# fatimp/SIFT3D

Measured on AMD Instinct MI355X. Metric: Mvoxel/s detect+describe (float32 volume resident in HBM), higher is better.
Workload: dtype f32; 1 GPU; 512x512x512 float32 lattice-blob volume, detect+describe, default parameters (sigma0 1.6, sigma_n 1.15, 3 levels/octave); parallelism=single GPU

## Files before the change

include/sift3d_amd.h:

```cpp
#ifndef SIFT3D_AMD_H
#define SIFT3D_AMD_H

#include <stddef.h>
#include <stdint.h>

#include "sift3d/imtypes.h"

#ifdef __cplusplus
extern "C" {
#endif

#define SIFT3D_AMD_API __attribute__((visibility("default")))


SIFT3D_AMD_API int
sift3d_amd_detect_keypoints_device(sift3d_detector *det, const float *d_volume,
                                   int nx, int ny, int nz, double ux, double uy,
                                   double uz, sift3d_keypoint_store *store);

SIFT3D_AMD_API int
sift3d_amd_image_set_units(sift3d_image *im, double ux, double uy, double uz);

SIFT3D_AMD_API int
sift3d_amd_detector_set_cuboid_extrema(sift3d_detector *det, int on);
// ... 659 lines not shown
                           float *d_R, int32_t *d_keep, void *d_tab, uint32_t max_cand, int slot, void *stream);

typedef struct {
    float R[9];
    float cx, cy, cz;
    int32_t level;
    uint32_t row1;
    double sd;
} sift3d_hip_kp;

SIFT3D_AMD_API int
sift3d_hip_describe(const sift3d_hip_level *d_levels, const sift3d_hip_kp *d_kp,
                    uint32_t n, float *d_hist, void *stream);

SIFT3D_AMD_API size_t sift3d_hip_describe_wlut_floats(int nlevels);
SIFT3D_AMD_API int
sift3d_hip_describe_wlut(const sift3d_hip_level *d_levels, int nlevels, const sift3d_hip_kp *d_kp,
                         uint32_t n, float *d_hist, float *d_wlut, void *stream);
SIFT3D_AMD_API size_t sift3d_hip_describe_part_bytes(uint32_t n);
SIFT3D_AMD_API int
sift3d_hip_describe_parts(const sift3d_hip_level *d_levels, int nlevels, const sift3d_hip_kp *d_kp,
                          uint32_t n, uint32_t n_exact, float *d_hist, float *d_hist2, float *d_wlut,
                          void *d_part, void *stream);
SIFT3D_AMD_API int
sift3d_hip_describe_clock(const float *d_wlut, int nlevels, int exact, uint64_t *cycles, uint64_t *ticks,
                          void *stream);
SIFT3D_AMD_API int
sift3d_hip_describe_wlut2(const sift3d_hip_level *d_levels, int nlevels, const sift3d_hip_kp *d_kp,
                          uint32_t n, float *d_hist, float *d_hist2, float *d_wlut, void *stream);
SIFT3D_AMD_API int
sift3d_hip_describe_ex(const sift3d_hip_level *d_levels, int nlevels, const sift3d_hip_kp *d_kp, uint32_t n,
                       uint32_t n_exact, float *d_hist, float *d_hist2, float *d_wlut, void *stream);

SIFT3D_AMD_API int sift3d_hip_slab_count(const sift3d_hip_cand *d_cand, const int32_t *d_keep, uint32_t n,
                                         int ngl, int K, int nkey, int32_t *d_cnt, void *stream);
SIFT3D_AMD_API size_t sift3d_hip_slab_pack_scratch_bytes(uint32_t n);
SIFT3D_AMD_API int sift3d_hip_slab_pack(const sift3d_hip_level *d_levels, const sift3d_hip_cand *d_cand,
                                        const int32_t *d_keep, const float *d_R, uint32_t n, int ngl,
                                        float *d_vals, void *d_recs, void *d_scratch, void *stream);
SIFT3D_AMD_API int sift3d_hip_slab_build(const void *d_all, size_t blk_bytes, size_t roff, size_t toff,
                                         int world, int nkey, const uint32_t *d_tab, uint32_t tot_k,
                                         uint32_t tot_c, void *d_out, void *stream);

#define SIFT3D_HIP_FACE_FLOATS 19
SIFT3D_AMD_API int
sift3d_hip_set_mesh(const float *faces );
// ... 18 lines not shown
```

sift3d_amd/csrc/sift3d_describe.hip:

```cpp
#include "sift3d_kernels_common.h"
#include "sift3d_math.h"

#include <algorithm>
#include <cmath>
#include <cstdlib>

struct FaceRec {
    float v0[3], e1[3], e2[3], t[3], q[3], e2q, idx[3];
};
static_assert(sizeof(FaceRec) == SIFT3D_HIP_FACE_FLOATS * 4, "face record layout");

__constant__ float c_face16[20 * 16];
__constant__ int c_bin_off[12];
__constant__ int c_oct_face[32];

constexpr int DQ = 256;
constexpr int HIST_USED = 800;
constexpr int HIST_LDS = 800;
constexpr int FACE_STRIDE = 20;
constexpr int RSUPER = 68;
constexpr int REC_FLOATS = 7 * RSUPER;
constexpr int rec_row(int r) { return r < 7 ? r * RSUPER : (r - 7) * RSUPER + 32; }
constexpr int rec_group(int r) { return (rec_row(r) / 4) % 16; }
constexpr bool rec_groups_distinct()
// ... 86 lines not shown
    int e;
    const float mant = frexpf(L.ux, &e);
    const float u2 = L.ux * L.ux;
    const bool ok = L.ux == L.uy && L.ux == L.uz && mant == 0.5f &&
                    rad2 / u2 < (float)(WL_STRIDE - WL_HEAD - 1) && u2 * (float)WL_STRIDE < 16777216.0f;
    if (threadIdx.x == 0) {
        tab[0] = ok ? 1.0f : 0.0f;
        tab[1] = 0.0f;
        tab[2] = __int_as_float((int)(__double_as_longlong(L.sd) & 0xffffffffll));
        tab[3] = __int_as_float((int)(__double_as_longlong(L.sd) >> 32));
    }
    if (!ok)
        return;
    for (int k = threadIdx.x; k < WL_STRIDE - WL_HEAD; k += 256) {
        const float sq = (float)k * u2;
        const float arg = -0.5f * sq / sig2;
        tab[WL_HEAD + k] = arg >= -150.0f ? s3d_expf(arg) : 0.0f;
    }
}

constexpr int DWAVES = 4;
constexpr int DPARTS = 4;

template <bool EXACT>
__global__ __launch_bounds__(64 * DWAVES) void k_describe(const sift3d_hip_level *__restrict__ levels,
                                                 const sift3d_hip_kp *__restrict__ kps, uint32_t first,
                                                 uint32_t n,
                                                 float *__restrict__ out, float *__restrict__ out2,
                                                 const float *__restrict__ wlut,
                                                 uint32_t *__restrict__ work, float *__restrict__ part,
                                                 uint32_t *__restrict__ done DESC_ABLATE_ARG)
{
    __shared__ float hist_[DWAVES][2 * HIST_LDS];
    __shared__ __attribute__((aligned(16))) float rec_[DWAVES][REC_FLOATS];
    __shared__ int queue_[DWAVES][DQ];
    __shared__ __attribute__((aligned(16))) float sface[20 * FACE_STRIDE];
    __shared__ int soct[32];
    __shared__ uint64_t sexp[32];
    const int wv = __builtin_amdgcn_readfirstlane((int)(threadIdx.x >> 6));
    const int lane = threadIdx.x & 63;
    float *const hist = hist_[wv];
    float *const rec = rec_[wv];
    const uint32_t rec_m0 = (uint32_t)__builtin_amdgcn_readfirstlane((int)lds_addr(rec));
    const uint32_t hist_m0 = (uint32_t)__builtin_amdgcn_readfirstlane((int)lds_addr(hist));
    int *const queue = queue_[wv];
    for (int i = threadIdx.x; i < 20 * 16; i += 64 * DWAVES)
        sface[(i >> 4) * FACE_STRIDE + (i & 15)] = c_face16[i];
    if (threadIdx.x < 32) {
        soct[threadIdx.x] = c_oct_face[threadIdx.x];
        sexp[threadIdx.x] = s3d_exp2_tab[threadIdx.x];
    }
    __syncthreads();
    const bool probe = work && blockIdx.x == 0 && threadIdx.x == 0;
    long long probe_c0 = 0, probe_w0 = 0;
    if (probe) {
        probe_c0 = clock64();
        probe_w0 = wall_clock64();
    }
    const bool split = !EXACT && part != nullptr;
    for (bool first_pass = true;; first_pass = false) {
    uint32_t item;
    if (work) {
        uint32_t t = 0;
        if (lane == 0)
            t = atomicAdd(work, 1u);
        item = (uint32_t)__builtin_amdgcn_readfirstlane((int)t);
    } else {
        if (!first_pass)
            break;
        item = blockIdx.x * DWAVES + wv;
    }
    const uint32_t ki = first + (split ? item / DPARTS : item);
    const int pp = split ? (int)(item % DPARTS) : 0;
    if (ki >= n)
        break;
    static_assert(2 * HIST_LDS == 25 * 64, "histogram clear: 25 whole-wave stores");
#define Z4(o) "ds_write_addtid_b32 %0 offset:" #o "\n\tds_write_addtid_b32 %0 offset:" #o "+256\n\t" \
              "ds_write_addtid_b32 %0 offset:" #o "+512\n\tds_write_addtid_b32 %0 offset:" #o "+768\n\t"
    asm volatile("s_mov_b32 m0, %1\n\ts_nop 0\n\t" Z4(0) Z4(1024) Z4(2048) Z4(3072) Z4(4096) Z4(5120)
                 "ds_write_addtid_b32 %0 offset:6144" ::"v"(0.0f), "s"(hist_m0) : "m0", "memory");
#undef Z4
    wave_sync();
    const sift3d_hip_kp K = kps[ki];
    const sift3d_hip_level L = levels[K.level];
    const uint32_t orow = K.row1 ? K.row1 - 1 : ki;
    const float *__restrict__ wtab = nullptr;
    const int icx = (int)K.cx, icy = (int)K.cy, icz = (int)K.cz;
    if (wlut) {
        const float *tab = wlut + (size_t)K.level * WL_STRIDE;
        const long long sdbits = ((long long)__float_as_int(tab[3]) << 32) | (unsigned)__float_as_int(tab[2]);
        if (tab[0] == 1.0f && sdbits == __double_as_longlong(K.sd) && (float)icx == K.cx &&
            (float)icy == K.cy && (float)icz == K.cz)
            wtab = tab + WL_HEAD;
    }

    typedef const float __attribute__((address_space(1))) *gfloat_p;
    const gfloat_p wsrc = wtab ? (gfloat_p)wtab : (gfloat_p) reinterpret_cast<const float *>(levels);
    const int wmask = wtab ? -1 : 0;

    const float sigma = (float)(K.sd * 7.071067812);
    const float rad = (float)(2.0 * (double)sigma);
    const float half_w = (float)((double)rad / 1.4142135623730951);
    const float desc_w = 2.0f * half_w;
    const float hist_w = desc_w / 4.0f;
    const float bin_f = 1.0f / hist_w;
    const float rad2 = rad * rad;
    const float sig2 = sigma * sigma;
    const float *R = K.R;
    const float iux = 1.0f / L.ux, iuy = 1.0f / L.uy, iuz = 1.0f / L.uz;
    Box B;
    bounds_f(K.cx, rad, L.ux, L.nx, B.xs, B.xe);
    bounds_f(K.cy, rad, L.uy, L.ny, B.ys, B.ye);
    bounds_f(K.cz, rad, L.uz, L.nz_glob, B.zs, B.ze);
    B.zs = max(B.zs, L.z_off + 1);
    B.ze = min(B.ze, L.z_off + L.nz - 2);
    const int xsh = 32 - __builtin_clz((unsigned)max(B.xe - B.xs, 1));
    const int ysh = xsh + 32 - __builtin_clz((unsigned)max(B.ye - B.ys, 1));
    const uint32_t xmask = (1u << xsh) - 1u, ymask = (1u << (ysh - xsh)) - 1u;
#if defined(__HIP_DEVICE_COMPILE__) && !defined(__gfx942__) && !defined(__gfx950__)
#error "k_describe's commit routes its factors with DPP quad_perm on wave64: validated on gfx942 / gfx950 only"
#endif
    const int half = lane >> 5, l5 = lane & 31;
    const int pc = l5 >> 2, pt = l5 & 3, pj = pt < 3 ? pt : 0;
    const int pxr = pt == 0 ? pc : 8 + pj;
    const int pdx = (pc >> 2) & 1, pdy = (pc >> 1) & 1, pdz = pc & 1;
    const int corner4 = 4 * (pdx + 4 * pdy + 16 * pdz);
    const int coff_a = corner4 + (EXACT ? (half == 0 ? 0 : HIST_LDS * 4) : half * (HIST_LDS * 4));
    const int coff_b = corner4 + (half == 1 ? 0 : HIST_LDS * 4);
    (void)coff_b;
    const unsigned long long lt_mask = (1ull << lane) - 1ull;

    uint32_t qhead = 0, qtail = 0;
    bool pend = false;
#ifdef SIFT3D_AMD_DIAG
    unsigned diag_voxels = 0;
#endif

    auto window = [&](int x, int y, int z, float &sq, float &vbx, float &vby, float &vbz) -> bool {
        const float dx = ((float)x - K.cx) * L.ux;
        const float dy = ((float)y - K.cy) * L.uy;
        const float dz = ((float)z - K.cz) * L.uz;
        sq = dx * dx + dy * dy + dz * dz;
        const float kx = R[0] * dx + R[3] * dy + R[6] * dz;
        const float ky = R[1] * dx + R[4] * dy + R[7] * dz;
        const float kz = R[2] * dx + R[5] * dy + R[8] * dz;
        vbx = (kx + half_w) * bin_f;
        vby = (ky + half_w) * bin_f;
        vbz = (kz + half_w) * bin_f;
        const float lo = fminf(fminf(vbx, vby), vbz), hi = fmaxf(fmaxf(vbx, vby), vbz);
        return !(sq > rad2) && !(lo < 0.0f) && !(hi >= 4.0f);
    };

    float pv[7] = { 0.f, 0.f, 0.f, 0.f, 0.f, 0.f, 0.f };
    int ppk = 0;
    const gfloat_p gdata = (gfloat_p)L.data;
    const uint32_t ys32 = (uint32_t)L.nx, zs32 = (uint32_t)L.nx * (uint32_t)L.ny;
    auto prefetch_loads = [&](uint32_t start, int cnt) {
        const int qv = queue[(start + lane) & (DQ - 1)];
        ppk = lane < cnt ? qv : ppk;
        const int x = B.xs + (int)((uint32_t)ppk & xmask), y = B.ys + (int)(((uint32_t)ppk >> xsh) & ymask),
                  zl = B.zs + (int)((uint32_t)ppk >> ysh) - L.z_off;
        const gfloat_p p = gdata + ((uint64_t)zs32 * (uint32_t)zl + (uint32_t)(x + (int)ys32 * y));
        pv[0] = p[1]; pv[1] = *(p - 1); pv[2] = p[ys32]; pv[3] = *(p - ys32);
        pv[4] = p[zs32]; pv[5] = *(p - zs32);
        if (wtab) {
            const int i = x - icx, j = y - icy, l = B.zs + (int)((uint32_t)ppk >> ysh) - icz;
            pv[6] = wtab[i * i + j * j + l * l];
        }
    };
    auto prefetch_weight = [&]() {
        if (wtab)
            return;
        const int x = B.xs + (int)((uint32_t)ppk & xmask), y = B.ys + (int)(((uint32_t)ppk >> xsh) & ymask);
        const float dx = ((float)x - K.cx) * L.ux;
        const float dy = ((float)y - K.cy) * L.uy;
        const float dz = ((float)(B.zs + (int)((uint32_t)ppk >> ysh)) - K.cz) * L.uz;
        pv[6] = s3d_expf_in_range(-0.5f * (dx * dx + dy * dy + dz * dz) / sig2, sexp);
    };
    auto prefetch = [&](uint32_t start, int cnt) {
        prefetch_loads(start, cnt);
        prefetch_weight();
    };

    float rp[2][7] = { { 0.f, 0.f, 0.f, 0.f, 0.f, 0.f, 0.f }, { 0.f, 0.f, 0.f, 0.f, 0.f, 0.f, 0.f } };
    const float *const xrd = rec + rec_row(pxr) + 16 * half;
    const int *const ard = reinterpret_cast<const int *>(rec + rec_row(11 + pj) + 16 * half);
    auto commit_write = [&](int pass) {
#define RS(i) "ds_write_addtid_b32 %" #i " offset:%c8*" #i "\n\t"
        asm volatile("s_mov_b32 m0, %7\n\ts_nop 0\n\t" RS(0) RS(1) RS(2) RS(3) RS(4) RS(5) RS(6)
                     ::"v"(rp[pass][0]), "v"(rp[pass][1]), "v"(rp[pass][2]), "v"(rp[pass][3]), "v"(rp[pass][4]),
                       "v"(rp[pass][5]), "v"(rp[pass][6]), "s"(rec_m0), "n"(RSUPER * 4)
                     : "m0", "memory");
#undef RS
        wave_sync();
    };
#define SB() __builtin_amdgcn_sched_barrier(0)
#ifndef DESC_OPT
#define DESC_OPT 7
#endif
#define QUAD_X(v) __int_as_float(__builtin_amdgcn_update_dpp(0, __float_as_int(v), 0x03, 0xf, 0xf, true))
#if DESC_OPT & 1
#define COMMIT_ADD(old, x) (EXACT ? (old) + QUAD_X(x) * (x) : quad_fmac(old, x))
#else
#define COMMIT_ADD(old, x) ((old) + QUAD_X(x) * (x))
#endif
#define KEEP(v) asm volatile("" ::"v"(v))
#define COMMIT_BEGIN(coff)                                                                    \
    const int coff4 = (coff);                                                                 \
    int4 cb4 = *reinterpret_cast<const int4 *>(ard);                                          \
    float4 cx4 = *reinterpret_cast<const float4 *>(xrd);                                      \
    int4 nb4 = cb4;                                                                           \
    float4 nx4 = cx4;
#define ROUND(u, ...)                                                                         \
    {                                                                                         \
        if (((u) & 3) == 0 && (u) + 4 < 16) {                                                 \
            nb4 = *reinterpret_cast<const int4 *>(ard + (u) + 4);                             \
            nx4 = *reinterpret_cast<const float4 *>(xrd + (u) + 4);                           \
        }                                                                                     \
        const int mb_[4] = { cb4.x, cb4.y, cb4.z, cb4.w };                                    \
        const float xv_[4] = { cx4.x, cx4.y, cx4.z, cx4.w };                                  \
        float *bin_ = reinterpret_cast<float *>(reinterpret_cast<char *>(hist) + (mb_[(u) & 3] + coff4)); \
        float old_ = 0.0f;                                                                    \
        if (!DESC_ABLATE(1))                                                                  \
            old_ = *bin_;                                                                     \
        SB();                                                                                 \
        { __VA_ARGS__ }                                                                       \
        SB();                                                                                 \
        if (!DESC_ABLATE(1))                                                                  \
            *bin_ = COMMIT_ADD(old_, xv_[(u) & 3]);                     \
        if (((u) & 3) == 3) {                                                                 \
            cb4 = nb4;                                                                        \
            cx4 = nx4;                                                                        \
        }                                                                                     \
        SB();                                                                                 \
    }
#define CHAIN_B()                                                                             \
    if (EXACT) {                                                                              \
        COMMIT_BEGIN(coff_b);                                                                 \
        ROUND(0, ) ROUND(1, ) ROUND(2, ) ROUND(3, ) ROUND(4, ) ROUND(5, ) ROUND(6, ) ROUND(7, ) \
        ROUND(8, ) ROUND(9, ) ROUND(10, ) ROUND(11, ) ROUND(12, ) ROUND(13, ) ROUND(14, ) ROUND(15, ) \
    }
    auto batch = [&](int cnt, const float *cv, int pk, uint32_t nstart, int ncnt) {
#ifdef SIFT3D_AMD_DIAG
        diag_voxels += (unsigned)cnt;
#endif
        if (DESC_ABLATE(2)) { prefetch(nstart, ncnt); return; }
        int x, y, z;
        float dx, dy, dz, kx, ky, kz, vbx, vby, vbz, gx, gy, gz, rx, ry, rz, m2;
        float t1, t2, t3, px, py, pz, det, di, kk;
        float4 A0, A1, A2, A3;
        int f0;
        bool live = false, found = false;
        int fidx = 0;
        float b0 = 0.f, b1 = 0.f, b2 = 0.f;
        commit_write(0);
        {
            COMMIT_BEGIN(coff_a);
            ROUND(0, x = B.xs + (int)((uint32_t)pk & xmask); y = B.ys + (int)(((uint32_t)pk >> xsh) & ymask);
                     z = B.zs + (int)((uint32_t)pk >> ysh);
                     dx = ((float)x - K.cx) * L.ux; KEEP(dx);)
            ROUND(1, dy = ((float)y - K.cy) * L.uy; dz = ((float)z - K.cz) * L.uz; KEEP(dy); KEEP(dz);
                     gx = 0.5f * (cv[0] - cv[1]); gy = 0.5f * (cv[2] - cv[3]); gz = 0.5f * (cv[4] - cv[5]);)
            ROUND(2, gx *= iux; gy *= iuy; gz *= iuz;
                     gx = gx * cv[6]; gy = gy * cv[6]; gz = gz * cv[6];)
            ROUND(3, kx = R[0] * dx + R[3] * dy + R[6] * dz; ky = R[1] * dx + R[4] * dy + R[7] * dz; KEEP(kx); KEEP(ky);)
            ROUND(4, kz = R[2] * dx + R[5] * dy + R[8] * dz;
                     vbx = (kx + half_w) * bin_f; vby = (ky + half_w) * bin_f; vbz = (kz + half_w) * bin_f;
                     KEEP(vbx); KEEP(vby); KEEP(vbz);)
            ROUND(5, rx = R[0] * gx + R[3] * gy + R[6] * gz; ry = R[1] * gx + R[4] * gy + R[7] * gz;)
            ROUND(6, rz = R[2] * gx + R[5] * gy + R[8] * gz; m2 = rx * rx + ry * ry + rz * rz;
                     live = lane < cnt && !(m2 < 1.1920928955078125e-06f);)
#if DESC_OPT & 2
            ROUND(7, const float g = 1.6180339887f, g2 = 2.6180339887f;
                     const float ax_ = fabsf(rx), ay_ = fabsf(ry), az_ = fabsf(rz);
                     t1 = __builtin_fmaf(g2, ay_, __builtin_fmaf(-g, az_, ax_));
                     t2 = __builtin_fmaf(g2, az_, __builtin_fmaf(-g, ax_, ay_));
                     t3 = __builtin_fmaf(g2, ax_, __builtin_fmaf(-g, ay_, az_));)
#else
            ROUND(7, const float g = 1.6180339887f, g2 = 2.6180339887f;
                     const float ax_ = fabsf(rx), ay_ = fabsf(ry), az_ = fabsf(rz);
                     t1 = ax_ + g2 * ay_ - g * az_; t2 = ay_ + g2 * az_ - g * ax_; t3 = az_ + g2 * ax_ - g * ay_;)
#endif
            ROUND(8, const int n1 = t1 < 0.0f, n2 = t2 < 0.0f, n3 = t3 < 0.0f;
                     const int cls = n1 + (1 - n1) * (2 * n2 + (1 - n2) * 3 * n3);
// ... 25 lines not shown
                    found = true;
                    open = false;
                }
                if (__ballot(open) == 0ull)
                    break;
            }
        }
        commit_write(1);
        {
            COMMIT_BEGIN(coff_a);
            int nx_, ny_, nzl_, qv_;
            gfloat_p np_;
            float mag, fx, fy, fz;
            int ix, iy, iz, cell4;
            float ax[2], ay[2], az[2], fld[14];
            ROUND(0, qv_ = queue[(nstart + lane) & (DQ - 1)];)
            ROUND(1, ppk = lane < ncnt ? qv_ : ppk;
                     nx_ = B.xs + (int)((uint32_t)ppk & xmask); ny_ = B.ys + (int)(((uint32_t)ppk >> xsh) & ymask);
                     nzl_ = B.zs + (int)((uint32_t)ppk >> ysh) - L.z_off;
                     np_ = gdata + ((uint64_t)zs32 * (uint32_t)nzl_ + (uint32_t)(nx_ + (int)ys32 * ny_));)
            ROUND(2, pv[0] = np_[1]; pv[1] = *(np_ - 1); pv[2] = np_[ys32]; pv[3] = *(np_ - ys32);)
            ROUND(3, pv[4] = np_[zs32]; pv[5] = *(np_ - zs32);
                     const int i = nx_ - icx; const int j = ny_ - icy; const int l = B.zs + (int)((uint32_t)ppk >> ysh) - icz;
                     pv[6] = wsrc[(i * i + j * j + l * l) & wmask];)
#if DESC_OPT & 2
            ROUND(4, mag = EXACT ? sqrtf(m2) : __builtin_amdgcn_sqrtf(m2);
                     mag = live && found ? mag : 0.0f;)
#else
            ROUND(4, mag = sqrtf(m2); mag = live && found ? mag : 0.0f;)
#endif
            ROUND(5, fx = vbx - floorf(vbx); fy = vby - floorf(vby); fz = vbz - floorf(vbz);
                     ix = (int)vbx; iy = (int)vby; iz = (int)vbz;)
            ROUND(6, const bool lx = ix >= 3; const bool ly = iy >= 3; const bool lz = iz >= 3;
                     ax[0] = lx ? 0.0f : 1.0f - fx; ax[1] = lx ? 1.0f - fx : fx;
                     ay[0] = ly ? 0.0f : 1.0f - fy; ay[1] = ly ? 1.0f - fy : fy;
                     az[0] = lz ? 0.0f : 1.0f - fz; az[1] = lz ? 1.0f - fz : fz;)
            ROUND(7, _Pragma("unroll") for (int c = 0; c < 4; c++)
                         fld[c] = mag * (ax[(c >> 2) & 1] * ay[(c >> 1) & 1] * az[c & 1]);)
            ROUND(8, _Pragma("unroll") for (int c = 4; c < 8; c++)
                         fld[c] = mag * (ax[(c >> 2) & 1] * ay[(c >> 1) & 1] * az[c & 1]);)
            ROUND(9, cell4 = 4 * (min(max(ix, 0), 2) + 4 * min(max(iy, 0), 2) + 16 * min(max(iz, 0), 2));
                     const bool ok = live && found;
                     fld[8] = ok ? b0 : 0.0f; fld[9] = ok ? b1 : 0.0f; fld[10] = ok ? b2 : 0.0f;)
            ROUND(10, _Pragma("unroll") for (int j = 0; j < 3; j++)
                          fld[11 + j] = __int_as_float(4 * ((fidx >> (10 * j)) & 1023) + cell4);)
            ROUND(11, _Pragma("unroll") for (int i = 0; i < 4; i++) {
                          const auto r = __builtin_amdgcn_permlane32_swap(__float_as_uint(fld[i]), __float_as_uint(fld[7 + i]), false, false);
// ... 87 lines not shown
            if (__builtin_expect(__ballot(cheap2(xx, yy, in0, in1)) != 0ull, 0)) {
                float sq, vbx, vby, vbz;
                in0 = window(pxs + xx, pys + yy, z, sq, vbx, vby, vbz);
                in1 = window(pxs + xx + 1, pys + yy, z, sq, vbx, vby, vbz);
            }
#else
            float sq, vbx, vby, vbz;
            bool in0 = window(pxs + xx, pys + yy, z, sq, vbx, vby, vbz);
            bool in1 = window(pxs + xx + 1, pys + yy, z, sq, vbx, vby, vbz);
#endif
            in0 = in0 && c0 + 2 * lane < ppe;
            in1 = in1 && c0 + 2 * lane < ppe && xx + 1 < pbx;
            const int pk0 = (int)((uint32_t)(ox + xx) | ((uint32_t)(oy + yy) << xsh) | ((uint32_t)(z - B.zs) << ysh));
            const int pk1 = pk0 + 1;
            xx += r128;
            yy += q128;
            if (xx >= pbe) {
                xx -= pbe;
                yy++;
            }
            const unsigned long long m0 = __ballot(in0), m1 = __ballot(in1);
            if ((m0 | m1) == 0ull)
                continue;
            const uint32_t before = (uint32_t)__popcll(m0 & lt_mask) + (uint32_t)__popcll(m1 & lt_mask);
            if (in0)
                queue[(qtail + before) & (DQ - 1)] = pk0;
            if (in1)
                queue[(qtail + before + (in0 ? 1u : 0u)) & (DQ - 1)] = pk1;
            qtail += (uint32_t)__popcll(m0) + (uint32_t)__popcll(m1);
            wave_sync();
            while (qtail - qhead >= 64) {
                if (pend) {
                    float cv[7];
#pragma unroll
                    for (int k = 0; k < 7; k++)
                        cv[k] = pv[k];
                    const int cpk = ppk;
                    batch(64, cv, cpk, qhead, 64);
                } else {
                    prefetch(qhead, 64);
                    pend = true;
                }
                qhead += 64;
            }
        }
    }
    {
// ... 68 lines not shown
            for (int o = 32; o > 0; o >>= 1)
                norm += __shfl_xor(norm, o, 64);
        }
        norm = sqrt(norm) + 2.220446049250313e-16;
        const float inv = (float)(1.0 / norm);
        wave_sync();
        for (int i = lane; i < HIST_USED; i += 64) {
            float el = hist[i] * inv;
            if (pass == 0)
                el = el < trunc ? el : trunc;
            hist[i] = el;
        }
        wave_sync();
    }
    for (int i = lane; i < 768; i += 64) {
        const float v = hist[c_bin_off[i % 12] + i / 12];
        out[(size_t)orow * 768 + i] = v;
        if (out2)
            out2[(size_t)orow * 768 + i] = v;
    }
    wave_sync();
    }
    if (probe) {
        unsigned long long *slot = reinterpret_cast<unsigned long long *>(work - (EXACT ? 0 : 1) + (EXACT ? 4 : 8));
        slot[0] = (unsigned long long)(clock64() - probe_c0);
        slot[1] = (unsigned long long)(wall_clock64() - probe_w0);
    }
}

__constant__ int c_face_vert[20];

constexpr int DB_TX = 64, DB_TY = 4;

__device__ __forceinline__ void dense_bin_one(const float *sface, const int *soct, const int *svert, float gx,
                                              float gy, float gz, float &w0, float &w1, float &w2, int &vid)
{
    const float m2 = gx * gx + gy * gy + gz * gz;
    w0 = 0.0f; w1 = 0.0f; w2 = 0.0f; vid = 0;
    if (m2 < 1.1920928955078125e-06f)
        return;
    float b0, b1, b2;
    int fi, f = soct[icos_guess(gx, gy, gz)];
    bool found = face_eval(reinterpret_cast<const float4 *>(sface + f * FACE_STRIDE), gx, gy, gz, b0, b1, b2, fi) &&
                 fminf(b0, fminf(b1, b2)) > 2e-5f;
    if (!found) {
        for (f = 0; f < 20; f++)
            if (face_eval(reinterpret_cast<const float4 *>(sface + f * FACE_STRIDE), gx, gy, gz, b0, b1, b2, fi)) {
// ... 515 lines not shown
static unsigned describe_grid(uint32_t count, bool counted)
{
    const unsigned need = (count + DWAVES - 1) / DWAVES;
    if (!counted)
        return need;
    static int cus = 0;
    if (!cus) {
        int dev = 0;
        hipDeviceProp_t prop;
        if (hipGetDevice(&dev) == hipSuccess && hipGetDeviceProperties(&prop, dev) == hipSuccess)
            cus = prop.multiProcessorCount;
        if (cus < 1)
            cus = 256;
    }
    const unsigned cap = (unsigned)cus * 4u;
    return need < cap ? need : cap;
}

size_t sift3d_hip_describe_part_bytes(uint32_t n)
{
    return n ? (size_t)n * DPARTS * HIST_USED * sizeof(float) + (size_t)n * sizeof(uint32_t) : 0;
}

static int describe_launch(const sift3d_hip_level *d_levels, int nlevels, const sift3d_hip_kp *d_kp, uint32_t n,
                           uint32_t n_exact, float *d_hist, float *d_hist2, const float *d_wlut,
                           void *d_part, void *stream)
{
    if (n_exact > n)
        n_exact = n;
#ifdef SIFT3D_AMD_DIAG
    static int ablate = getenv("SIFT3D_AMD_DESC_ABLATE") ? atoi(getenv("SIFT3D_AMD_DESC_ABLATE")) : 0;
#define DESC_ABLATE_PASS , ablate
#else
#define DESC_ABLATE_PASS
#endif
    uint32_t *work = d_wlut ? reinterpret_cast<uint32_t *>(const_cast<float *>(d_wlut) + (size_t)nlevels * WL_STRIDE)
                            : nullptr;
    if (n_exact) {
        hipLaunchKernelGGL(k_describe<true>, dim3(describe_grid(n_exact, work != nullptr)), dim3(64 * DWAVES), 0,
                           (hipStream_t)stream, d_levels, d_kp, 0u, n_exact, d_hist, d_hist2, d_wlut,
                           work, (float *)nullptr, (uint32_t *)nullptr DESC_ABLATE_PASS);
        LAUNCH_CHECK();
    }
    if (n > n_exact) {
        const uint32_t nf = n - n_exact;
        void *tmp = nullptr;
        if (!d_part) {
            HIPCHK(hipMalloc(&tmp, sift3d_hip_describe_part_bytes(nf)));
            d_part = tmp;
        }
        float *parts = reinterpret_cast<float *>(d_part);
        uint32_t *done = reinterpret_cast<uint32_t *>(parts + (size_t)nf * DPARTS * HIST_USED);
        hipError_t e = hipMemsetAsync(done, 0, (size_t)nf * sizeof(uint32_t), (hipStream_t)stream);
        if (e == hipSuccess) {
            hipLaunchKernelGGL(k_describe<false>, dim3(describe_grid(nf * DPARTS, work != nullptr)),
                               dim3(64 * DWAVES), 0, (hipStream_t)stream, d_levels, d_kp, n_exact, n, d_hist,
                               d_hist2, d_wlut, work ? work + 1 : nullptr, parts, done DESC_ABLATE_PASS);
            e = hipGetLastError();
        }
        if (tmp) {
            const hipError_t e2 = hipStreamSynchronize((hipStream_t)stream);
            (void)hipFree(tmp);
            if (e == hipSuccess)
                e = e2;
        }
        if (e != hipSuccess)
            return fail("k_describe", e, __FILE__, __LINE__);
    }
#undef DESC_ABLATE_PASS
    return SIFT3D_SUCCESS;
}

int sift3d_hip_describe(const sift3d_hip_level *d_levels, const sift3d_hip_kp *d_kp, uint32_t n,
                        float *d_hist, void *stream)
{
    if (!n)
        return SIFT3D_SUCCESS;
    return describe_launch(d_levels, 0, d_kp, n, 0, d_hist, nullptr, nullptr, nullptr, stream);
}

int sift3d_hip_describe_parts(const sift3d_hip_level *d_levels, int nlevels, const sift3d_hip_kp *d_kp,
                              uint32_t n, uint32_t n_exact, float *d_hist, float *d_hist2, float *d_wlut,
                              void *d_part, void *stream)
{
    if (!n)
        return SIFT3D_SUCCESS;
    if (!d_wlut || nlevels < 1)
        return describe_launch(d_levels, 0, d_kp, n, n_exact, d_hist, d_hist2, nullptr, d_part, stream);
    hipLaunchKernelGGL(k_desc_wlut, dim3(nlevels), dim3(256), 0, (hipStream_t)stream, d_levels, nlevels,
                       d_wlut);
    return describe_launch(d_levels, nlevels, d_kp, n, n_exact, d_hist, d_hist2, d_wlut, d_part, stream);
}

int sift3d_hip_describe_ex(const sift3d_hip_level *d_levels, int nlevels, const sift3d_hip_kp *d_kp,
                           uint32_t n, uint32_t n_exact, float *d_hist, float *d_hist2, float *d_wlut,
                           void *stream)
{
    return sift3d_hip_describe_parts(d_levels, nlevels, d_kp, n, n_exact, d_hist, d_hist2, d_wlut, nullptr,
                                     stream);
}

int sift3d_hip_describe_clock(const float *d_wlut, int nlevels, int exact, uint64_t *cycles, uint64_t *ticks,
                              void *stream)
{
    if (!d_wlut || nlevels < 1 || !cycles || !ticks)
        return SIFT3D_FAILURE;
    uint64_t v[2] = { 0, 0 };
    const uint32_t *ctr = reinterpret_cast<const uint32_t *>(d_wlut + (size_t)nlevels * WL_STRIDE);
    HIPCHK(hipMemcpyAsync(v, ctr + (exact ? 4 : 8), sizeof(v), hipMemcpyDeviceToHost, (hipStream_t)stream));
    HIPCHK(hipStreamSynchronize((hipStream_t)stream));
    *cycles = v[0];
    *ticks = v[1];
    return SIFT3D_SUCCESS;
}
// ... 131 lines not shown
```

sift3d_amd/csrc/sift3d_detect.c:

```c

static int require_device(void)
{
    if (!sift3d_amd_device_available()) {
        ERR("sift3d_amd: no HIP device is available; this library has no CPU path \n");
        return SIFT3D_FAILURE;
    }
    return SIFT3D_SUCCESS;
}

static int ensure_device(sift3d_detector *d)
{
    int i;
    if (d->stream) {
        if (sift3d_hip_current_device() != d->device) {
            ERR("sift3d_amd: this detector belongs to HIP device %d, the current device is %d \n",
                d->device, sift3d_hip_current_device());
            return SIFT3D_FAILURE;
        }
        return SIFT3D_SUCCESS;
    }
    if (require_device())
        return SIFT3D_FAILURE;
    d->device = sift3d_hip_current_device();
    if (!(d->stream = sift3d_hip_stream_create()) || !(d->oct_stream = sift3d_hip_stream_create_high()) ||
// ... 791 lines not shown
    return SIFT3D_SUCCESS;
}

enum { DESC_LV_MAX = 32 };

static int ensure_kp_list(sift3d_detector *d, int num)
{
    if ((uint32_t)num > d->kp_cap) {
        const uint32_t cap = (uint32_t)num + (uint32_t)num / 4 + 256;
        sift3d_hip_host_free(d->h_kp);
        d->kp_cap = 0;
        d->h_kp = (sift3d_hip_kp *)sift3d_hip_host_alloc(sizeof(sift3d_hip_kp) * (size_t)cap);
        if (!d->h_kp)
            return SIFT3D_FAILURE;
        d->kp_cap = cap;
    }
    if (d->ngl > DESC_LV_MAX) {
        ERR("sift3d_amd: at most %d Gaussian levels per octave are supported \n", DESC_LV_MAX);
        return SIFT3D_FAILURE;
    }
    return SIFT3D_SUCCESS;
}

static inline int desc_bucket(const sift3d_detector *d, const keypoint_t *k)
{
    return k->s + 1 + (exact_desc_keypoint(d->exact_desc, k->sd, k->o, d->units) ? 0 : d->ngl);
}

static size_t order_keypoints(sift3d_detector *d, const sift3d_keypoint_store *kp)
{
    const size_t num = kp->num;
    const int nt = host_threads(num), nlv = d->ngl;
    size_t cnt[HOST_THREADS_MAX][2 * DESC_LV_MAX], start[HOST_THREADS_MAX][2 * DESC_LV_MAX];
    size_t n_exact = 0;
    memset(cnt, 0, sizeof(cnt));
#pragma omp parallel num_threads(nt)
    {
        const int nth = omp_get_num_threads(), t = omp_get_thread_num();
        const size_t lo = num * t / nth, hi = num * (t + 1) / nth;
        size_t q;
        for (q = lo; q < hi; q++)
            cnt[t][desc_bucket(d, kp->buf + q)]++;
#pragma omp barrier
#pragma omp single
        {
            size_t pos = 0;
            int b, u;
            for (b = 0; b < 2 * nlv; b++) {
                const int bk = b < nlv ? nlv - 1 - b : 3 * nlv - 1 - b;
                if (b == nlv)
                    n_exact = pos;
                for (u = 0; u < nth; u++) {
                    start[u][bk] = pos;
                    pos += cnt[u][bk];
                }
            }
        }
        for (q = lo; q < hi; q++) {
            const keypoint_t *k = kp->buf + q;
            sift3d_hip_kp *r = d->h_kp + start[t][desc_bucket(d, k)]++;
            memcpy(r->R, k->R, sizeof(r->R));
            r->cx = (float)k->xd;
            r->cy = (float)k->yd;
            r->cz = (float)k->zd;
            r->level = k->o * d->ngl + k->s + 1;
            r->row1 = (uint32_t)q + 1u;
            r->sd = k->sd;
        }
    }
    return n_exact;
}

static int ensure_descriptor_store(const sift3d_detector *d, sift3d_descriptor_store *desc, size_t num)
{
    desc->nx = d->odims[0][0];
    desc->ny = d->odims[0][1];
    desc->nz = d->odims[0][2];
    if (!desc->pinned || num > desc->cap) {
        const size_t cap = num + num / 8 + 64;
        desc_store_release(desc);
        desc->hist = (float *)sift3d_hip_host_alloc(sizeof(float) * DESC_NUMEL * cap);
        desc->xyzsd = (double *)malloc(sizeof(double) * 4 * cap);
        if (!desc->hist || !desc->xyzsd) {
            desc->pinned = desc->hist != NULL;
            desc_store_release(desc);
            return SIFT3D_FAILURE;
        }
        desc->pinned = 1;
        desc->cap = cap;
    }
    desc->num = num;
    desc->d_num = 0;
    if (desc->keep_device && num > desc->d_cap) {
        sift3d_hip_free(desc->d_hist);
        desc->d_cap = 0;
        desc->d_hist = (float *)sift3d_hip_malloc(sizeof(float) * DESC_NUMEL * desc->cap);
        if (!desc->d_hist)
            return SIFT3D_FAILURE;
        desc->d_cap = desc->cap;
    }
    return SIFT3D_SUCCESS;
}

int sift3d_extract_descriptors(sift3d_detector *const d, const sift3d_keypoint_store *const kp,
                               sift3d_descriptor_store *const desc)
{
    const int num = (int)kp->num;
    const double t_start = now_s();
    int i;
    size_t n_exact;
    uint64_t rng;

    if (verify_keys(d, kp) || check_window_packing(d, kp) || ensure_kp_list(d, num))
        return SIFT3D_FAILURE;
    n_exact = order_keypoints(d, kp);
    if (ensure_descriptor_store(d, desc, (size_t)num))
        return SIFT3D_FAILURE;
    d->t_pending &= ~2;
    rng = range_start("sift3d: descriptors");
    sift3d_hip_event_record(d->ev[6], d->stream);
    {
        float *dev_view = (float *)sift3d_hip_host_device_ptr(desc->hist);
        const sift3d_hip_kp *kp_view = (const sift3d_hip_kp *)sift3d_hip_host_device_ptr(d->h_kp);
        const size_t need = sift3d_hip_describe_part_bytes((uint32_t)(num - (int)n_exact));
        if (need > d->dpart_bytes) {
            sift3d_hip_free(d->d_dpart);
            d->dpart_bytes = 0;
            d->d_dpart = sift3d_hip_malloc(need + need / 8);
            if (!d->d_dpart)
                return SIFT3D_FAILURE;
            d->dpart_bytes = need + need / 8;
        }
        if (!dev_view || !kp_view ||
            sift3d_hip_describe_parts(d->d_levels, d->num_octaves * d->ngl, kp_view, (uint32_t)num,
                                      (uint32_t)n_exact, dev_view, desc->keep_device ? desc->d_hist : NULL,
                                      d->d_wlut, need ? d->d_dpart : NULL, d->stream))
            return SIFT3D_FAILURE;
    }
    sift3d_hip_event_record(d->ev[7], d->stream);
    for (i = 0; i < num; i++) {
        const keypoint_t *k = kp->buf + i;
        const double f = ldexp(1.0, k->o);
        desc->xyzsd[4 * (size_t)i] = k->xd * f;
        desc->xyzsd[4 * (size_t)i + 1] = k->yd * f;
        desc->xyzsd[4 * (size_t)i + 2] = k->zd * f;
        desc->xyzsd[4 * (size_t)i + 3] = k->sd;
    }
    if (sift3d_hip_stream_sync(d->stream))
        return SIFT3D_FAILURE;
    range_stop(rng);
    if (desc->keep_device)
        desc->d_num = (size_t)num;
    d->t_pending |= 2;
    d->t[T_DESCRIBE_WALL] = now_s() - t_start;
    return SIFT3D_SUCCESS;
}
```

Before: 4289 Mvoxel/s.

## Add lattice-keypoint describe path with specialized kernel and mbcnt prefix counts

Keypoints whose centers sit on integer voxel positions with isotropic power-of-two units and a matching level scale are sorted into a third bucket and described by a LATTICE specialization of the kernel. That path always uses the precomputed Gaussian weight table and rebuilds the offsets dx/dy/dz from the integer weight indices instead of recomputing coordinates. DESC_OPT also turns on an LDS commit pipeline that uses direct LDS pointers with precomputed addresses, and mbcnt-based ballot prefix counts. The cost is an extra kernel launch, more host-side bucketing, and more code variants. A VALU microbenchmark is added as well.

```diff
diff --git a/include/sift3d_amd.h b/include/sift3d_amd.h
--- a/include/sift3d_amd.h
+++ b/include/sift3d_amd.h
@@ -705,6 +705,11 @@
 sift3d_hip_describe_parts(const sift3d_hip_level *d_levels, int nlevels, const sift3d_hip_kp *d_kp,
                           uint32_t n, uint32_t n_exact, float *d_hist, float *d_hist2, float *d_wlut,
                           void *d_part, void *stream);
+SIFT3D_AMD_API int sift3d_hip_describe_lattice_level(float ux, float uy, float uz, double sd);
+SIFT3D_AMD_API int
+sift3d_hip_describe_lattice(const sift3d_hip_level *d_levels, int nlevels, const sift3d_hip_kp *d_kp,
+                            uint32_t n, uint32_t n_exact, uint32_t n_lattice, float *d_hist, float *d_hist2,
+                            float *d_wlut, void *d_part, void *stream);
 SIFT3D_AMD_API int
 sift3d_hip_describe_clock(const float *d_wlut, int nlevels, int exact, uint64_t *cycles, uint64_t *ticks,
                           void *stream);
diff --git a/profiles/microbench/valu_rate.hip b/profiles/microbench/valu_rate.hip
--- /dev/null
+++ b/profiles/microbench/valu_rate.hip
@@ -0,0 +1,73 @@
+#include <hip/hip_runtime.h>
+#include <cstdint>
+#include <cstdio>
+#include <cstdlib>
+#define CHK(x) do{hipError_t e=(x); if(e!=hipSuccess){printf("err %s line %d\n", hipGetErrorString(e), __LINE__); exit(1);} }while(0)
+
+template <int OP>
+__global__ __launch_bounds__(256) void k(double *out, int iters, int seed)
+{
+    uint32_t a[8];
+    uint64_t w[8];
+    float f[8];
+    for (int i = 0; i < 8; i++) {
+        a[i] = (uint32_t)(seed + i + threadIdx.x);
+        w[i] = a[i];
+        f[i] = 1.0f + 0.001f * (float)a[i];
+    }
+    const uint32_t m = 3u + seed;
+    const float fm = 1.0000001f, fc = 1e-9f;
+    for (int it = 0; it < iters; it++) {
+#pragma unroll
+        for (int r = 0; r < 4; r++) {
+#pragma unroll
+            for (int i = 0; i < 8; i++) {
+                if (OP == 0) asm volatile("v_fma_f32 %0, %0, %1, %2" : "+v"(f[i]) : "v"(fm), "v"(fc));
+                if (OP == 1) asm volatile("v_mul_lo_u32 %0, %0, %1" : "+v"(a[i]) : "v"(m));
+                if (OP == 2) asm volatile("v_mad_u64_u32 %0, vcc, %1, %2, %0" : "+v"(w[i]) : "v"(a[i]), "v"(m) : "vcc");
+                if (OP == 3) asm volatile("v_mul_u32_u24 %0, %0, %1" : "+v"(a[i]) : "v"(m));
+                if (OP == 4) asm volatile("v_mad_i32_i24 %0, %0, %1, %0" : "+v"(a[i]) : "v"(m));
+                if (OP == 5) asm volatile("v_lshl_add_u64 %0, %1, 2, %0" : "+v"(w[i]) : "v"(w[(i + 1) & 7]));
+                if (OP == 6) asm volatile("v_rcp_f32 %0, %0" : "+v"(f[i]));
+                if (OP == 7) asm volatile("v_sqrt_f32 %0, %0" : "+v"(f[i]));
+                if (OP == 8) asm volatile("v_cvt_f32_i32 %0, %1" : "=v"(f[i]) : "v"(a[i]));
+            }
+        }
+    }
+    double s = 0;
+    for (int i = 0; i < 8; i++) s += (double)a[i] + (double)w[i] + f[i];
+    out[blockIdx.x * 256 + threadIdx.x] = s;
+}
+
+template <int OP> void run(const char *name, double *d_o)
+{
+    for (int bpc = 1; bpc <= 8; bpc *= 2) {
+        const int iters = 4000;
+        hipEvent_t e0, e1; CHK(hipEventCreate(&e0)); CHK(hipEventCreate(&e1));
+        float ms = 0;
+        for (int rep = 0; rep < 2; rep++) {
+            CHK(hipEventRecord(e0));
+            hipLaunchKernelGGL((k<OP>), dim3(256 * bpc), dim3(256), 0, 0, d_o, iters, 1);
+            CHK(hipEventRecord(e1)); CHK(hipEventSynchronize(e1));
+            CHK(hipEventElapsedTime(&ms, e0, e1));
+        }
+        const double instr_per_simd = (double)bpc * iters * 32;
+        printf("%-16s %d waves/SIMD: %8.3f ms -> %6.2f cycles / instruction / SIMD (2.4 GHz)\n", name, bpc, ms,
+               ms * 1e-3 * 2.4e9 / instr_per_simd);
+    }
+}
+
+int main()
+{
+    double *d_o; CHK(hipMalloc(&d_o, 256 * 8 * 256 * 8));
+    run<0>("v_fma_f32", d_o);
+    run<1>("v_mul_lo_u32", d_o);
+    run<2>("v_mad_u64_u32", d_o);
+    run<3>("v_mul_u32_u24", d_o);
+    run<4>("v_mad_i32_i24", d_o);
+    run<5>("v_lshl_add_u64", d_o);
+    run<6>("v_rcp_f32", d_o);
+    run<7>("v_sqrt_f32", d_o);
+    run<8>("v_cvt_f32_i32", d_o);
+    return 0;
+}
diff --git a/sift3d_amd/csrc/sift3d_describe.hip b/sift3d_amd/csrc/sift3d_describe.hip
--- a/sift3d_amd/csrc/sift3d_describe.hip
+++ b/sift3d_amd/csrc/sift3d_describe.hip
@@ -132,7 +132,7 @@
 constexpr int DWAVES = 4;
 constexpr int DPARTS = 4;
 
-template <bool EXACT>
+template <bool EXACT, bool LATTICE = false>
 __global__ __launch_bounds__(64 * DWAVES) void k_describe(const sift3d_hip_level *__restrict__ levels,
                                                  const sift3d_hip_kp *__restrict__ kps, uint32_t first,
                                                  uint32_t n,
@@ -158,7 +158,8 @@
         sface[(i >> 4) * FACE_STRIDE + (i & 15)] = c_face16[i];
     if (threadIdx.x < 32) {
         soct[threadIdx.x] = c_oct_face[threadIdx.x];
-        sexp[threadIdx.x] = s3d_exp2_tab[threadIdx.x];
+        if (!LATTICE)
+            sexp[threadIdx.x] = s3d_exp2_tab[threadIdx.x];
     }
     __syncthreads();
     const bool probe = work && blockIdx.x == 0 && threadIdx.x == 0;
@@ -196,7 +197,9 @@
     const uint32_t orow = K.row1 ? K.row1 - 1 : ki;
     const float *__restrict__ wtab = nullptr;
     const int icx = (int)K.cx, icy = (int)K.cy, icz = (int)K.cz;
-    if (wlut) {
+    if (LATTICE) {
+        wtab = wlut + (size_t)K.level * WL_STRIDE + WL_HEAD;
+    } else if (wlut) {
         const float *tab = wlut + (size_t)K.level * WL_STRIDE;
         const long long sdbits = ((long long)__float_as_int(tab[3]) << 32) | (unsigned)__float_as_int(tab[2]);
         if (tab[0] == 1.0f && sdbits == __double_as_longlong(K.sd) && (float)icx == K.cx &&
@@ -205,8 +208,9 @@
     }
 
     typedef const float __attribute__((address_space(1))) *gfloat_p;
-    const gfloat_p wsrc = wtab ? (gfloat_p)wtab : (gfloat_p) reinterpret_cast<const float *>(levels);
-    const int wmask = wtab ? -1 : 0;
+    const bool have_tab = LATTICE || wtab;
+    const gfloat_p wsrc = have_tab ? (gfloat_p)wtab : (gfloat_p) reinterpret_cast<const float *>(levels);
+    const int wmask = have_tab ? -1 : 0;
 
     const float sigma = (float)(K.sd * 7.071067812);
     const float rad = (float)(2.0 * (double)sigma);
@@ -238,7 +242,6 @@
     const int coff_a = corner4 + (EXACT ? (half == 0 ? 0 : HIST_LDS * 4) : half * (HIST_LDS * 4));
     const int coff_b = corner4 + (half == 1 ? 0 : HIST_LDS * 4);
     (void)coff_b;
-    const unsigned long long lt_mask = (1ull << lane) - 1ull;
 
     uint32_t qhead = 0, qtail = 0;
     bool pend = false;
@@ -263,6 +266,7 @@
 
     float pv[7] = { 0.f, 0.f, 0.f, 0.f, 0.f, 0.f, 0.f };
     int ppk = 0;
+    int pwi = 0, pwj = 0, pwl = 0;
     const gfloat_p gdata = (gfloat_p)L.data;
     const uint32_t ys32 = (uint32_t)L.nx, zs32 = (uint32_t)L.nx * (uint32_t)L.ny;
     auto prefetch_loads = [&](uint32_t start, int cnt) {
@@ -276,10 +280,11 @@
         if (wtab) {
             const int i = x - icx, j = y - icy, l = B.zs + (int)((uint32_t)ppk >> ysh) - icz;
             pv[6] = wtab[i * i + j * j + l * l];
+            pwi = i; pwj = j; pwl = l;
         }
     };
     auto prefetch_weight = [&]() {
-        if (wtab)
+        if (LATTICE || wtab)
             return;
         const int x = B.xs + (int)((uint32_t)ppk & xmask), y = B.ys + (int)(((uint32_t)ppk >> xsh) & ymask);
         const float dx = ((float)x - K.cx) * L.ux;
@@ -306,7 +311,7 @@
     };
 #define SB() __builtin_amdgcn_sched_barrier(0)
 #ifndef DESC_OPT
-#define DESC_OPT 7
+#define DESC_OPT 111
 #endif
 #define QUAD_X(v) __int_as_float(__builtin_amdgcn_update_dpp(0, __float_as_int(v), 0x03, 0xf, 0xf, true))
 #if DESC_OPT & 1
@@ -315,6 +320,49 @@
 #define COMMIT_ADD(old, x) ((old) + QUAD_X(x) * (x))
 #endif
 #define KEEP(v) asm volatile("" ::"v"(v))
+#if (DESC_OPT & 64)
+typedef __attribute__((address_space(3))) float *lds_float_p;
+#define LDS_F32(a) (*(lds_float_p)(uintptr_t)(uint32_t)(a))
+#define OFFCHAIN (!EXACT)
+#define CHUNK_ADDR(q)                                                                         \
+    aq_[q] = make_int4(bq_[q].x + coffh, bq_[q].y + coffh, bq_[q].z + coffh, bq_[q].w + coffh); \
+    KEEP(aq_[q].x); KEEP(aq_[q].y); KEEP(aq_[q].z); KEEP(aq_[q].w);
+#define COMMIT_BEGIN(coff)                                                                    \
+    const int coffh = (coff) + (int)lds_addr(hist);                                           \
+    int4 bq_[2], aq_[2];                                                                      \
+    float4 xq_[2];                                                                            \
+    bq_[0] = *reinterpret_cast<const int4 *>(ard);                                            \
+    xq_[0] = *reinterpret_cast<const float4 *>(xrd);                                          \
+    bq_[1] = bq_[0];                                                                          \
+    xq_[1] = xq_[0];                                                                          \
+    CHUNK_ADDR(0)                                                                             \
+    aq_[1] = aq_[0];
+#define ROUND(u, ...)                                                                         \
+    {                                                                                         \
+        constexpr int cur_ = ((u) >> 2) & 1, nxt_ = cur_ ^ 1;                                 \
+        const int mb_[4] = { bq_[cur_].x, bq_[cur_].y, bq_[cur_].z, bq_[cur_].w };            \
+        const int ma_[4] = { aq_[cur_].x, aq_[cur_].y, aq_[cur_].z, aq_[cur_].w };            \
+        const float xv_[4] = { xq_[cur_].x, xq_[cur_].y, xq_[cur_].z, xq_[cur_].w };          \
+        const int addr_ = OFFCHAIN ? ma_[(u) & 3] : mb_[(u) & 3] + coffh;                     \
+        float old_ = 0.0f;                                                                    \
+        if (!DESC_ABLATE(1))                                                                  \
+            old_ = LDS_F32(addr_);                                                            \
+        SB();                                                                                 \
+        if (((u) & 3) == 0 && (u) + 4 < 16) {                                                 \
+            bq_[nxt_] = *reinterpret_cast<const int4 *>(ard + (u) + 4);                       \
+            xq_[nxt_] = *reinterpret_cast<const float4 *>(xrd + (u) + 4);                     \
+            SB();                                                                             \
+        }                                                                                     \
+        { __VA_ARGS__ }                                                                       \
+        if (OFFCHAIN && ((u) & 3) == 1 && (u) + 3 < 16) {                                     \
+            CHUNK_ADDR(nxt_)                                                                  \
+        }                                                                                     \
+        SB();                                                                                 \
+        if (!DESC_ABLATE(1))                                                                  \
+            LDS_F32(addr_) = COMMIT_ADD(old_, xv_[(u) & 3]);            \
+        SB();                                                                                 \
+    }
+#else
 #define COMMIT_BEGIN(coff)                                                                    \
     const int coff4 = (coff);                                                                 \
     int4 cb4 = *reinterpret_cast<const int4 *>(ard);                                          \
@@ -344,6 +392,7 @@
         }                                                                                     \
         SB();                                                                                 \
     }
+#endif
 #define CHAIN_B()                                                                             \
     if (EXACT) {                                                                              \
         COMMIT_BEGIN(coff_b);                                                                 \
@@ -366,10 +415,18 @@
         commit_write(0);
         {
             COMMIT_BEGIN(coff_a);
-            ROUND(0, x = B.xs + (int)((uint32_t)pk & xmask); y = B.ys + (int)(((uint32_t)pk >> xsh) & ymask);
-                     z = B.zs + (int)((uint32_t)pk >> ysh);
-                     dx = ((float)x - K.cx) * L.ux; KEEP(dx);)
-            ROUND(1, dy = ((float)y - K.cy) * L.uy; dz = ((float)z - K.cz) * L.uz; KEEP(dy); KEEP(dz);
+            ROUND(0, if (LATTICE && (DESC_OPT & 8)) {
+                         dx = (float)pwi * L.ux; dy = (float)pwj * L.uy; dz = (float)pwl * L.uz;
+                         KEEP(dy); KEEP(dz);
+                     } else {
+                         x = B.xs + (int)((uint32_t)pk & xmask); y = B.ys + (int)(((uint32_t)pk >> xsh) & ymask);
+                         z = B.zs + (int)((uint32_t)pk >> ysh);
+                         dx = ((float)x - K.cx) * L.ux;
+                     }
+                     KEEP(dx);)
+            ROUND(1, if (!(LATTICE && (DESC_OPT & 8))) {
+                         dy = ((float)y - K.cy) * L.uy; dz = ((float)z - K.cz) * L.uz; KEEP(dy); KEEP(dz);
+                     }
                      gx = 0.5f * (cv[0] - cv[1]); gy = 0.5f * (cv[2] - cv[3]); gz = 0.5f * (cv[4] - cv[5]);)
             ROUND(2, gx *= iux; gy *= iuy; gz *= iuz;
                      gx = gx * cv[6]; gy = gy * cv[6]; gz = gz * cv[6];)
@@ -441,7 +498,8 @@
             ROUND(2, pv[0] = np_[1]; pv[1] = *(np_ - 1); pv[2] = np_[ys32]; pv[3] = *(np_ - ys32);)
             ROUND(3, pv[4] = np_[zs32]; pv[5] = *(np_ - zs32);
                      const int i = nx_ - icx; const int j = ny_ - icy; const int l = B.zs + (int)((uint32_t)ppk >> ysh) - icz;
-                     pv[6] = wsrc[(i * i + j * j + l * l) & wmask];)
+                     pv[6] = wsrc[(i * i + j * j + l * l) & wmask];
+                     if (LATTICE && (DESC_OPT & 8)) { pwi = i; pwj = j; pwl = l; })
 #if DESC_OPT & 2
             ROUND(4, mag = EXACT ? sqrtf(m2) : __builtin_amdgcn_sqrtf(m2);
                      mag = live && found ? mag : 0.0f;)
@@ -575,7 +633,14 @@
             const unsigned long long m0 = __ballot(in0), m1 = __ballot(in1);
             if ((m0 | m1) == 0ull)
                 continue;
+#if DESC_OPT & 32
+            const uint32_t before = __builtin_amdgcn_mbcnt_hi(
+                (uint32_t)(m1 >> 32), __builtin_amdgcn_mbcnt_lo((uint32_t)m1, __builtin_amdgcn_mbcnt_hi(
+                (uint32_t)(m0 >> 32), __builtin_amdgcn_mbcnt_lo((uint32_t)m0, 0u))));
+#else
+            const unsigned long long lt_mask = (1ull << lane) - 1ull;
             const uint32_t before = (uint32_t)__popcll(m0 & lt_mask) + (uint32_t)__popcll(m1 & lt_mask);
+#endif
             if (in0)
                 queue[(qtail + before) & (DQ - 1)] = pk0;
             if (in1)
@@ -690,7 +755,8 @@
     wave_sync();
     }
     if (probe) {
-        unsigned long long *slot = reinterpret_cast<unsigned long long *>(work - (EXACT ? 0 : 1) + (EXACT ? 4 : 8));
+        unsigned long long *slot =
+            reinterpret_cast<unsigned long long *>(work - (EXACT ? 0 : LATTICE ? 2 : 1) + (EXACT ? 4 : 8));
         slot[0] = (unsigned long long)(clock64() - probe_c0);
         slot[1] = (unsigned long long)(wall_clock64() - probe_w0);
     }
@@ -1252,12 +1318,27 @@
     return n ? (size_t)n * DPARTS * HIST_USED * sizeof(float) + (size_t)n * sizeof(uint32_t) : 0;
 }
 
+int sift3d_hip_describe_lattice_level(float ux, float uy, float uz, double sd)
+{
+    const float sigma = (float)(sd * 7.071067812);
+    const float rad = (float)(2.0 * (double)sigma);
+    int e;
+    const float mant = frexpf(ux, &e);
+    const float rad2 = rad * rad, u2 = ux * ux;
+    return ux == uy && ux == uz && mant == 0.5f && ux >= 0.0009765625f && ux <= 1024.0f &&
+           rad2 / u2 < 0.999f * (float)(WL_STRIDE - WL_HEAD - 1) && u2 * (float)WL_STRIDE < 16777216.0f;
+}
+
 static int describe_launch(const sift3d_hip_level *d_levels, int nlevels, const sift3d_hip_kp *d_kp, uint32_t n,
-                           uint32_t n_exact, float *d_hist, float *d_hist2, const float *d_wlut,
-                           void *d_part, void *stream)
+                           uint32_t n_exact, uint32_t n_lattice, float *d_hist, float *d_hist2,
+                           const float *d_wlut, void *d_part, void *stream)
 {
     if (n_exact > n)
         n_exact = n;
+    if (!(DESC_OPT & 8) || !d_wlut)
+        n_lattice = 0;
+    if (n_lattice > n - n_exact)
+        return launch_fail("sift3d_hip_describe", "more lattice records than fast records");
 #ifdef SIFT3D_AMD_DIAG
     static int ablate = getenv("SIFT3D_AMD_DESC_ABLATE") ? atoi(getenv("SIFT3D_AMD_DESC_ABLATE")) : 0;
 #define DESC_ABLATE_PASS , ablate
@@ -1282,10 +1363,18 @@
         float *parts = reinterpret_cast<float *>(d_part);
         uint32_t *done = reinterpret_cast<uint32_t *>(parts + (size_t)nf * DPARTS * HIST_USED);
         hipError_t e = hipMemsetAsync(done, 0, (size_t)nf * sizeof(uint32_t), (hipStream_t)stream);
-        if (e == hipSuccess) {
-            hipLaunchKernelGGL(k_describe<false>, dim3(describe_grid(nf * DPARTS, work != nullptr)),
-                               dim3(64 * DWAVES), 0, (hipStream_t)stream, d_levels, d_kp, n_exact, n, d_hist,
-                               d_hist2, d_wlut, work ? work + 1 : nullptr, parts, done DESC_ABLATE_PASS);
+        const uint32_t ng = nf - n_lattice;
+        if (e == hipSuccess && ng) {
+            hipLaunchKernelGGL((k_describe<false, false>), dim3(describe_grid(ng * DPARTS, work != nullptr)),
+                               dim3(64 * DWAVES), 0, (hipStream_t)stream, d_levels, d_kp, n_exact, n - n_lattice,
+                               d_hist, d_hist2, d_wlut, work ? work + 1 : nullptr, parts, done DESC_ABLATE_PASS);
+            e = hipGetLastError();
+        }
+        if (e == hipSuccess && n_lattice) {
+            hipLaunchKernelGGL((k_describe<false, true>), dim3(describe_grid(n_lattice * DPARTS, true)),
+                               dim3(64 * DWAVES), 0, (hipStream_t)stream, d_levels, d_kp, n - n_lattice, n,
+                               d_hist, d_hist2, d_wlut, work + 2, parts + (size_t)ng * DPARTS * HIST_USED,
+                               done + ng DESC_ABLATE_PASS);
             e = hipGetLastError();
         }
         if (tmp) {
@@ -1306,20 +1395,29 @@
 {
     if (!n)
         return SIFT3D_SUCCESS;
-    return describe_launch(d_levels, 0, d_kp, n, 0, d_hist, nullptr, nullptr, nullptr, stream);
+    return describe_launch(d_levels, 0, d_kp, n, 0, 0, d_hist, nullptr, nullptr, nullptr, stream);
+}
+
+int sift3d_hip_describe_lattice(const sift3d_hip_level *d_levels, int nlevels, const sift3d_hip_kp *d_kp,
+                                uint32_t n, uint32_t n_exact, uint32_t n_lattice, float *d_hist, float *d_hist2,
+                                float *d_wlut, void *d_part, void *stream)
+{
+    if (!n)
+        return SIFT3D_SUCCESS;
+    if (!d_wlut || nlevels < 1)
+        return describe_launch(d_levels, 0, d_kp, n, n_exact, 0, d_hist, d_hist2, nullptr, d_part, stream);
+    hipLaunchKernelGGL(k_desc_wlut, dim3(nlevels), dim3(256), 0, (hipStream_t)stream, d_levels, nlevels,
+                       d_wlut);
+    return describe_launch(d_levels, nlevels, d_kp, n, n_exact, n_lattice, d_hist, d_hist2, d_wlut, d_part,
+                           stream);
 }
 
 int sift3d_hip_describe_parts(const sift3d_hip_level *d_levels, int nlevels, const sift3d_hip_kp *d_kp,
                               uint32_t n, uint32_t n_exact, float *d_hist, float *d_hist2, float *d_wlut,
                               void *d_part, void *stream)
 {
-    if (!n)
-        return SIFT3D_SUCCESS;
-    if (!d_wlut || nlevels < 1)
-        return describe_launch(d_levels, 0, d_kp, n, n_exact, d_hist, d_hist2, nullptr, d_part, stream);
-    hipLaunchKernelGGL(k_desc_wlut, dim3(nlevels), dim3(256), 0, (hipStream_t)stream, d_levels, nlevels,
-                       d_wlut);
-    return describe_launch(d_levels, nlevels, d_kp, n, n_exact, d_hist, d_hist2, d_wlut, d_part, stream);
+    return sift3d_hip_describe_lattice(d_levels, nlevels, d_kp, n, n_exact, 0, d_hist, d_hist2, d_wlut, d_part,
+                                       stream);
 }
 
 int sift3d_hip_describe_ex(const sift3d_hip_level *d_levels, int nlevels, const sift3d_hip_kp *d_kp,
diff --git a/sift3d_amd/csrc/sift3d_detect.c b/sift3d_amd/csrc/sift3d_detect.c
--- a/sift3d_amd/csrc/sift3d_detect.c
+++ b/sift3d_amd/csrc/sift3d_detect.c
@@ -837,17 +837,31 @@
     return SIFT3D_SUCCESS;
 }
 
+static inline int lattice_keypoint(const sift3d_detector *d, const keypoint_t *k)
+{
+    const sift3d_hip_level *L = d->h_levels + (k->o * d->ngl + k->s + 1);
+    const float c[3] = { (float)k->xd, (float)k->yd, (float)k->zd };
+    int a;
+    for (a = 0; a < 3; a++)
+        if (!(c[a] >= 0.0f && c[a] < 8388608.0f && (float)(int)c[a] == c[a]))
+            return 0;
+    return memcmp(&k->sd, &L->sd, sizeof(double)) == 0 &&
+           sift3d_hip_describe_lattice_level(L->ux, L->uy, L->uz, L->sd);
+}
+
 static inline int desc_bucket(const sift3d_detector *d, const keypoint_t *k)
 {
-    return k->s + 1 + (exact_desc_keypoint(d->exact_desc, k->sd, k->o, d->units) ? 0 : d->ngl);
-}
-
-static size_t order_keypoints(sift3d_detector *d, const sift3d_keypoint_store *kp)
+    if (exact_desc_keypoint(d->exact_desc, k->sd, k->o, d->units))
+        return k->s + 1;
+    return k->s + 1 + (lattice_keypoint(d, k) ? 2 : 1) * d->ngl;
+}
+
+static size_t order_keypoints(sift3d_detector *d, const sift3d_keypoint_store *kp, size_t *n_lattice)
 {
     const size_t num = kp->num;
     const int nt = host_threads(num), nlv = d->ngl;
-    size_t cnt[HOST_THREADS_MAX][2 * DESC_LV_MAX], start[HOST_THREADS_MAX][2 * DESC_LV_MAX];
-    size_t n_exact = 0;
+    size_t cnt[HOST_THREADS_MAX][3 * DESC_LV_MAX], start[HOST_THREADS_MAX][3 * DESC_LV_MAX];
+    size_t n_exact = 0, lattice_first = num;
     memset(cnt, 0, sizeof(cnt));
 #pragma omp parallel num_threads(nt)
     {
@@ -861,10 +875,12 @@
         {
             size_t pos = 0;
             int b, u;
-            for (b = 0; b < 2 * nlv; b++) {
-                const int bk = b < nlv ? nlv - 1 - b : 3 * nlv - 1 - b;
+            for (b = 0; b < 3 * nlv; b++) {
+                const int bk = b < nlv ? nlv - 1 - b : b < 2 * nlv ? 3 * nlv - 1 - b : 5 * nlv - 1 - b;
                 if (b == nlv)
                     n_exact = pos;
+                if (b == 2 * nlv)
+                    lattice_first = pos;
                 for (u = 0; u < nth; u++) {
                     start[u][bk] = pos;
                     pos += cnt[u][bk];
@@ -883,6 +899,7 @@
             r->sd = k->sd;
         }
     }
+    *n_lattice = num - lattice_first;
     return n_exact;
 }
 
@@ -923,12 +940,12 @@
     const int num = (int)kp->num;
     const double t_start = now_s();
     int i;
-    size_t n_exact;
+    size_t n_exact, n_lattice;
     uint64_t rng;
 
     if (verify_keys(d, kp) || check_window_packing(d, kp) || ensure_kp_list(d, num))
         return SIFT3D_FAILURE;
-    n_exact = order_keypoints(d, kp);
+    n_exact = order_keypoints(d, kp, &n_lattice);
     if (ensure_descriptor_store(d, desc, (size_t)num))
         return SIFT3D_FAILURE;
     d->t_pending &= ~2;
@@ -947,9 +964,10 @@
             d->dpart_bytes = need + need / 8;
         }
         if (!dev_view || !kp_view ||
-            sift3d_hip_describe_parts(d->d_levels, d->num_octaves * d->ngl, kp_view, (uint32_t)num,
-                                      (uint32_t)n_exact, dev_view, desc->keep_device ? desc->d_hist : NULL,
-                                      d->d_wlut, need ? d->d_dpart : NULL, d->stream))
+            sift3d_hip_describe_lattice(d->d_levels, d->num_octaves * d->ngl, kp_view, (uint32_t)num,
+                                        (uint32_t)n_exact, (uint32_t)n_lattice, dev_view,
+                                        desc->keep_device ? desc->d_hist : NULL, d->d_wlut,
+                                        need ? d->d_dpart : NULL, d->stream))
             return SIFT3D_FAILURE;
     }
     sift3d_hip_event_record(d->ev[7], d->stream);
```

Measured after the change: 4389 Mvoxel/s (median of 6 runs). 1.02x the previous value.
